# gk969/stm32-speech-recognition

Hardware: AMD Instinct MI355X
Metric: utterances/sec (256-frame, 100 templates) (higher is better)
Workload: dtype int32

## Files before the change

stm32_speech_recognition_amd/csrc/k_mfcc.hip:

```cpp
#include "sr_fft_dev.h"

#ifndef SR_MEL_CHUNKED
#define SR_MEL_CHUNKED 1
#endif

namespace sr {

constexpr int kMfccWaves = 4;
constexpr int kFramesPerWave = 16, kFramesPerWaveMid = 4, kFramesPerWaveSmall = 1;
#ifndef SR_MAG_TAB_BINS
#define SR_MAG_TAB_BINS 8
#endif
constexpr int mfcc_tab_bins(int fpw) { return fpw == kFramesPerWave ? SR_MAG_TAB_BINS : 0; }
static_assert(SR_MAG_TAB_BINS == 0 || SR_MAG_TAB_BINS == 4 || SR_MAG_TAB_BINS == 8, "table bins per lane");
constexpr int kMelPad = kMel + 1;
__device__ __forceinline__ constexpr int mel_chunk_word(int j) { return 256 * ((j >> 2) & 1) + 4 * ((j >> 3) ^ (4 * ((j >> 2) & 1))) + (j & 3); }
constexpr int mfcc_wave_lds_words(int fpw) { return kXchgWords + fpw * kMelPad + 64; }

template <typename Base>
struct MfccTabArgs : Base {
    const uint16_t *mag_q;
    uint32_t mag_table_off;
};
template <typename Base>
constexpr int mfcc_feat_kind<MfccTabArgs<Base>> = mfcc_feat_kind<Base>;
template <typename Base>
static MfccTabArgs<Base> mfcc_tab_args(const Base &b, const MfccMagTab &tab)
{
    MfccTabArgs<Base> r;
    static_cast<Base &>(r) = b;
    r.mag_q = tab.mag_q;
    r.mag_table_off = tab.mag_table_off;
    return r;
}

template <int kFPW, typename Args = MfccTabArgs<MfccArgs>>
__global__ void __launch_bounds__(64 * kMfccWaves, 4) k_mfcc(const Args a)
{
    constexpr int kFeat = mfcc_feat_kind<Args>;
    constexpr uint32_t kFeatW = (kFeat == SR_FEAT_FFT || kFeat == SR_FEAT_MAG) ? kBins : kMel;
    constexpr int kWaveLdsWords = mfcc_wave_lds_words(kFPW);
    constexpr int kTabBins = mfcc_tab_bins(kFPW);
    extern __shared__ __attribute__((aligned(16))) uint32_t smem[];
    __shared__ uint32_t s_dctM[kCoef * kMelPad];
    __shared__ int s_dctS[kCoef * kMelPad];
    __shared__ u32x4 s_tw3[kTw3Row * 4], s_tw5[8 * 64];
    __shared__ u32x4 s_tm[4 * 64];
    const int lane = threadIdx.x & 63, w = __builtin_amdgcn_readfirstlane(threadIdx.x >> 6);
    uint32_t *buf = smem + w * kWaveLdsWords;
    uint32_t *xw = buf;
    uint32_t *powb = buf + kXchgWords, *moff = powb + kFPW * kMelPad;

    for (int i = threadIdx.x; i < kCoef * kMel; i += blockDim.x) {
        const int c = a.t.dct[i], o = (i / kMel) * kMelPad + i % kMel;
        s_dctM[o] = (uint32_t)(((c < 0 ? -c : c) * 262144 + 99) / 100);
        s_dctS[o] = (c > 0) - (c < 0);
    }
    __syncthreads();

    LaneTw tw;
    load_lane_tw(a.t, lane, tw);
    if (w == 0 && lane < 4) {
        const uint32_t *f = &tw.s3[0][0][0];
#pragma unroll
        for (int c = 0; c < 8; c++) s_tw3[lane * kTw3Row + c] = u32x4{f[4 * c], f[4 * c + 1], f[4 * c + 2], f[4 * c + 3]};
    }
    if (w == 1 % kMfccWaves) store_tw32(s_tw5, lane, tw.s5);
#ifndef SR_INJECT_LDS_RACE
    if (w == 2 % kMfccWaves) {
#pragma unroll
        for (int c = 0; c < 2; c++) {
            s_tm[64 * c + lane] = *(const u32x4 *)(a.t.tri_even_m + 8 * lane + 4 * c);
            s_tm[64 * (c + 2) + lane] = *(const u32x4 *)(a.t.tri_odd_m + 8 * lane + 4 * c);
        }
    }
#endif
    __syncthreads();
#ifdef SR_INJECT_LDS_RACE
    if (w == 2 % kMfccWaves) {
#if SR_INJECT_LDS_RACE >= 2
        __builtin_amdgcn_s_sleep(127);
#endif
#pragma unroll
        for (int c = 0; c < 2; c++) {
            s_tm[64 * c + lane] = *(const u32x4 *)(a.t.tri_even_m + 8 * lane + 4 * c);
            s_tm[64 * (c + 2) + lane] = *(const u32x4 *)(a.t.tri_odd_m + 8 * lane + 4 * c);
        }
    }
#endif
    int hamm_m[3];
#pragma unroll
    for (int k = 0; k < 3; k++) hamm_m[k] = (lane + 64 * k < kFrameLen) ? hamm_fused_multiplier(a.t.hamm[lane + 64 * k]) : 0;
    int f_lo = 0, p_hi = 0, p_lo = 0, x_hi = 0, x_lo = 0;
    if (lane < kMel) {
        const int h = lane;
        f_lo = (h == 0) ? 0 : (int)a.t.tri_cen[h - 1];
        const int f_hi = (h == kMel - 1) ? kBins : (int)a.t.tri_cen[h + 1];
        const int ih = f_hi - 1, il = f_lo ? f_lo - 1 : 0, half = (h & 1) ? kBins : 0;
#if SR_MEL_CHUNKED
        p_hi = half + mel_chunk_word(ih), x_hi = (ih >> 3) > 0 ? (ih >> 3) - 1 : 0;
        p_lo = half + mel_chunk_word(il), x_lo = (il >> 3) > 0 ? (il >> 3) - 1 : 0;
#else
        p_hi = half + ih, x_hi = (ih >> 3) > 0 ? (ih >> 3) - 1 : 0;
        p_lo = half + il, x_lo = (il >> 3) > 0 ? (il >> 3) - 1 : 0;
#endif
    }
    const uint64_t mag_p = (uint64_t)a.mag_q;
    const u32x4 mag_rs = {(uint32_t)mag_p, (uint32_t)(mag_p >> 32) | (2u << 16), kMagTabEntries, 0x00027000u};
    const uint32_t tw_off = 32u * (uint32_t)lane;
#if SR_MEL_CHUNKED
    const int e_base = mel_chunk_word(lane);
    constexpr int kEs = 32, kEh = 128;
    const int c0 = mel_chunk_word(8 * lane), c1 = mel_chunk_word(8 * lane + 4);
#else
    const int e_base = lane;
    constexpr int kEs = 64, kEh = 256;
    const int c0 = 8 * lane, c1 = 8 * lane + 4;
#endif

    uint32_t item = blockIdx.x;
    uint32_t nx_nfrm = 0;
    int nx_mid = 0, nx_seg0 = 0;
    if (item < a.n_items) {
        const sr_vad_rec *rec = a.vad + item / a.tiles;
        nx_nfrm = rec->frm_num;
        nx_mid = (int)rec->atap.mid_val;
        nx_seg0 = rec->seg[0];
    }
    for (; item < a.n_items; item += gridDim.x) {
        const uint32_t b = item / a.tiles, tile = item - b * a.tiles;
        const uint32_t nfrm = nx_nfrm;
        const int mid = nx_mid, seg0 = nx_seg0;
        if (item + gridDim.x < a.n_items) {
            const sr_vad_rec *rec = a.vad + (item + gridDim.x) / a.tiles;
            nx_nfrm = rec->frm_num;
            nx_mid = (int)rec->atap.mid_val;
            nx_seg0 = rec->seg[0];
        }
        const uint16_t *row = a.pcm + (uint64_t)b * a.pcm_stride;
        int16_t *out = a.mfcc + (uint64_t)b * a.max_frames * kCoef;
        const uint32_t f0 = tile * (kMfccWaves * kFPW) + w * kFPW;
        uint32_t *frow = nullptr;
        if constexpr (kFeat != 0) frow = a.feat + (uint64_t)b * a.max_frames * kFeatW;
        uint32_t nf = 0;
        if (f0 < nfrm) nf = (nfrm - f0 < (uint32_t)kFPW) ? nfrm - f0 : (uint32_t)kFPW;

        uint32_t s_pp[3] = {0, 0, 0};
        if (nf) {
            const uint16_t *x = row + seg0 + (int)kHop * (int)f0;
#pragma unroll
            for (int k = 0; k < 3; k++) {
                const int i = lane + 64 * k;
                if (i < kFrameLen) s_pp[k] = *(const u32_align2 *)(x + i - 1);
            }
        }
        for (uint32_t fi = 0; fi < nf; fi++) {
#pragma unroll
            for (int k = 0; k < 3; k++) {
                const int i = lane + 64 * k;
                if (i < kFrameLen) xw[i] = k == 0 ? window_sample<4>(s_pp[k], mid, hamm_m[k]) : window_sample<2>(s_pp[k], mid, hamm_m[k]);
            }
            if (fi + 1 < nf) {
                const uint16_t *x = row + seg0 + (int)kHop * (int)(f0 + fi + 1);
#pragma unroll
                for (int k = 0; k < 3; k++) {
                    const int i = lane + 64 * k;
                    if (i < kFrameLen) s_pp[k] = *(const u32_align2 *)(x + i - 1);
                }
            }
            wave_sync();
            uint32_t v[4][4], u[4][4];
            fft_front_real160(xw, lane, tw, s_tw3, v);
            fft_exchange(buf, lane, v, u);
#pragma unroll
            for (int e4 = 0; e4 < 4; e4++)
                bfly_pk<false>(u[0][e4], u[1][e4], u[2][e4], u[3][e4], tw.s4[0][0], tw.s4[0][1], tw.s4[1][0], tw.s4[1][1],
                               tw.s4[2][0], tw.s4[2][1], tw.s4[3][0], tw.s4[3][1]);
            wave_sync();
            uint32_t k5[4][4][2];
            load_tw32(s_tw5, lane, k5);
            uint32_t nn[8];
#pragma unroll
            for (int e3 = 0; e3 < 4; e3++) {
                bfly_pk<true>(u[e3][0], u[e3][1], u[e3][2], u[e3][3], k5[e3][0][0], k5[e3][0][1], k5[e3][1][0],
                              k5[e3][1][1], k5[e3][2][0], k5[e3][2][1], k5[e3][3][0], k5[e3][3][1]);
                if constexpr (kFeat == SR_FEAT_FFT) {
                    uint32_t *fr = frow + (f0 + fi) * kFeatW + lane + 64 * e3;
                    fr[0] = u[e3][0];
                    fr[256] = u[e3][1];
                }
                nn[2 * e3] = (uint32_t)sdot2z(u[e3][0], u[e3][0]);
                nn[2 * e3 + 1] = (uint32_t)sdot2z(u[e3][1], u[e3][1]);
            }
            const uint32_t nmax = max(max(max(max(nn[0], nn[1]), nn[2]), max(max(nn[3], nn[4]), nn[5])), max(nn[6], nn[7]));
#ifdef SR_TESTING
            const bool quiet = __builtin_expect(__builtin_amdgcn_ballot_w64(nmax > kMagSmallMax) == 0 && !a.mag_table_off, 1);
#else
            const bool quiet = __builtin_expect(__builtin_amdgcn_ballot_w64(nmax > kMagSmallMax) == 0, 1);
#endif
            u32x4 tw_e[2], tw_o[2];
            bool cheap = true;
            if (!quiet) {
#pragma unroll
                for (int c = 0; c < 2; c++) {
                    tw_e[c] = *(const u32x4 *)((const char *)a.t.tri_even32 + tw_off + 16 * c);
                    tw_o[c] = *(const u32x4 *)((const char *)a.t.tri_odd32 + tw_off + 16 * c);
                }
                cheap = __builtin_amdgcn_ballot_w64(nmax > a.mag_cheap_max) == 0;
            } else {
                asm volatile("" : "=v"(tw_e[0]), "=v"(tw_e[1]), "=v"(tw_o[0]), "=v"(tw_o[1]));
            }
            uint32_t *eb = buf + e_base;
            if (kTabBins > 0 && quiet) {
                uint32_t tq[8];
#pragma unroll
                for (int e3 = 0; e3 < 4; e3++) {
                    if constexpr (kTabBins == 8)
                        asm volatile("buffer_load_ushort %0, %1, %2, 0 idxen" : "=v"(tq[2 * e3]) : "v"(nn[2 * e3]), "s"(mag_rs));
                    asm volatile("buffer_load_ushort %0, %1, %2, 0 idxen" : "=v"(tq[2 * e3 + 1]) : "v"(nn[2 * e3 + 1]), "s"(mag_rs));
                }
                uint32_t q0s[4];
                if constexpr (kTabBins == 4) {
#pragma unroll
                    for (int e3 = 0; e3 < 4; e3++) q0s[e3] = cvt_u32(__builtin_amdgcn_sqrtf((float)(int)nn[2 * e3]) * 10.0f) << 2;
                }
                if constexpr (kTabBins == 8)
                    asm volatile("s_waitcnt vmcnt(0)" : "+v"(tq[0]), "+v"(tq[1]), "+v"(tq[2]), "+v"(tq[3]), "+v"(tq[4]), "+v"(tq[5]), "+v"(tq[6]), "+v"(tq[7]));
                else
                    asm volatile("s_waitcnt vmcnt(0)" : "+v"(tq[1]), "+v"(tq[3]), "+v"(tq[5]), "+v"(tq[7]));
#pragma unroll
                for (int e3 = 0; e3 < 4; e3++) {
                    uint32_t q0, q1 = tq[2 * e3 + 1];
                    if constexpr (kTabBins == 8) q0 = tq[2 * e3];
                    else q0 = q0s[e3];
                    if constexpr (kFeat == SR_FEAT_MAG) {
                        uint32_t *fr = frow + (f0 + fi) * kFeatW + lane + 64 * e3;
                        fr[0] = q0 >> 2;
                        fr[256] = q1 >> 2;
                    }
                    eb[kEs * e3] = umul24(q0, q0);
                    eb[kEs * e3 + kEh] = umul24(q1, q1);
                }
            } else if (cheap) {
#pragma unroll
                for (int e3 = 0; e3 < 4; e3++) {
                    const f32x2 m = f32x2{__builtin_amdgcn_sqrtf((float)(int)nn[2 * e3]), __builtin_amdgcn_sqrtf((float)(int)nn[2 * e3 + 1])} *
                                    f32x2{10.0f, 10.0f};
                    const uint32_t m0 = cvt_u32(m.x), m1 = cvt_u32(m.y);
                    if constexpr (kFeat == SR_FEAT_MAG) {
                        uint32_t *fr = frow + (f0 + fi) * kFeatW + lane + 64 * e3;
                        fr[0] = m0;
                        fr[256] = m1;
                    }
                    eb[kEs * e3] = umul24(m0, m0);
                    eb[kEs * e3 + kEh] = umul24(m1, m1);
                }
            } else {
#pragma unroll
                for (int e3 = 0; e3 < 4; e3++) {
                    const f32x2 m = sqrt_rn_int2(f32x2{(float)(int)nn[2 * e3], (float)(int)nn[2 * e3 + 1]}) * f32x2{10.0f, 10.0f};
                    const uint32_t m0 = cvt_u32(m.x), m1 = cvt_u32(m.y);
                    if constexpr (kFeat == SR_FEAT_MAG) {
                        uint32_t *fr = frow + (f0 + fi) * kFeatW + lane + 64 * e3;
                        fr[0] = m0;
                        fr[256] = m1;
                    }
                    eb[kEs * e3] = umul24(m0, m0);
                    eb[kEs * e3 + kEh] = umul24(m1, m1);
                }
            }
            wave_sync();
            uint32_t pe[8], po[8], xe, xo;
            {
                const uint4 q0 = *(const uint4 *)(buf + c0), q1 = *(const uint4 *)(buf + c1);
                const uint32_t e[8] = {q0.x, q0.y, q0.z, q0.w, q1.x, q1.y, q1.z, q1.w};
                uint32_t se = 0, so = 0;
                if (quiet) {
#pragma unroll
                    for (int c = 0; c < 2; c++) {
                        const u32x4 me = s_tm[64 * c + lane], mo = s_tm[64 * (c + 2) + lane];
#pragma unroll
                        for (int k = 0; k < 4; k++) {
                            const uint32_t es = kTabBins > 0 ? e[4 * c + k] : e[4 * c + k] << 4;
                            se += mel_term_fused(es, me[k]);
                            so += mel_term_fused(es, mo[k]);
                            pe[4 * c + k] = se;
                            po[4 * c + k] = so;
                        }
                    }
                } else {
#pragma unroll
                    for (int c = 0; c < 2; c++) {
#pragma unroll
                        for (int k = 0; k < 4; k++) {
                            se += e[4 * c + k] * tw_e[c][k] / 100u;
                            so += e[4 * c + k] * tw_o[c][k] / 100u;
                            pe[4 * c + k] = se;
                            po[4 * c + k] = so;
                        }
                    }
                }
                xe = wave_scan_incl(se);
                xo = wave_scan_incl(so);
            }
            *(uint4 *)(buf + c0) = make_uint4(pe[0], pe[1], pe[2], pe[3]);
            *(uint4 *)(buf + c1) = make_uint4(pe[4], pe[5], pe[6], pe[7]);
            *(uint4 *)(buf + kBins + c0) = make_uint4(po[0], po[1], po[2], po[3]);
            *(uint4 *)(buf + kBins + c1) = make_uint4(po[4], po[5], po[6], po[7]);
            buf[2 * kBins + lane] = xe;
            moff[lane] = xo;
            wave_sync();
            if (lane < kMel) {
                const uint32_t *X = (lane & 1) ? moff : buf + 2 * kBins;
                const uint32_t hi = buf[p_hi] + X[x_hi], lo = f_lo ? buf[p_lo] + X[x_lo] : 0u;
                powb[fi * kMelPad + lane] = hi - lo;
                if constexpr (kFeat == SR_FEAT_MEL) frow[(f0 + fi) * kFeatW + lane] = hi - lo;
            }
            wave_sync();
        }

        {
            constexpr int kLogRounds = (kFPW * kMelPad + 63) / 64;
            const uint32_t n_log = nf * kMelPad;
            uint32_t nv[kLogRounds], mv[kLogRounds];
            u32x2 tv[kLogRounds];
#pragma unroll
            for (int r = 0; r < kLogRounds; r++) {
                const uint32_t t = lane + 64u * r;
                nv[r] = powb[t];
                mv[r] = log100_est(nv[r]);
                tv[r] = *(const u32_pair_align4 *)((const char *)a.t.log_thr + 4u * mv[r]);
            }
#pragma unroll
            for (int r = 0; r < kLogRounds; r++) {
                const uint32_t t = lane + 64u * r;
                if (t < n_log) powb[t] = log100_fix(nv[r], mv[r], tv[r].x, tv[r].y) << 14;
            }
        }
        wave_sync();
        if constexpr (kFeat == SR_FEAT_LOGMEL) {
            uint32_t *fw = frow + f0 * kFeatW;
            for (uint32_t t = lane; t < nf * kFeatW; t += 64) {
                const uint32_t fi = t / kFeatW, h = t - fi * kFeatW;
                fw[t] = powb[fi * kMelPad + h] >> 14;
            }
        }
        {
            int16_t *out_w = out + (size_t)f0 * kCoef;
#pragma unroll
            for (uint32_t t = lane; t < (uint32_t)(kFPW * kCoef); t += 64) {
                if (t < nf * kCoef) {
                    const uint32_t fi = umul24(t, 10923u) >> 17, h = t - umul24(fi, (uint32_t)kCoef);
                    const uint32_t *pw = powb + umul24(fi, (uint32_t)kMelPad), *dm = s_dctM + umul24(h, (uint32_t)kMelPad);
                    const int *ds = s_dctS + umul24(h, (uint32_t)kMelPad);
                    int acc = 0;
#pragma unroll
                    for (int i = 0; i < kMel; i++) acc = mad24((int)__umulhi(pw[i], dm[i]), ds[i], acc);
                    out_w[t] = (int16_t)acc;
                }
            }
        }
        wave_sync();
        {
            const uint32_t r0 = f0 + nf, r1 = (f0 + kFPW < a.max_frames) ? f0 + kFPW : a.max_frames;
            for (uint32_t t = r0 * kCoef + lane; t < r1 * kCoef && r0 < r1; t += 64) out[t] = 0;
        }
        if constexpr (kFeat != 0) {
            const uint32_t r0 = f0 + nf, r1 = (f0 + kFPW < a.max_frames) ? f0 + kFPW : a.max_frames;
            for (uint32_t t = r0 * kFeatW + lane; t < r1 * kFeatW && r0 < r1; t += 64) frow[t] = 0;
        }
    }
}

uint32_t mfcc_ext_frames_per_tile();
int mfcc_ext_occupancy(int *per_cu);
void launch_mfcc_ext(const MfccArgs &a, uint32_t grid, hipStream_t s);
void launch_mfcc_ext_features(const MfccArgs &a, int kind, uint32_t *feat, uint32_t grid, hipStream_t s);

uint32_t mfcc_frames_per_tile(uint32_t frame_len) { return frame_len == 320 ? mfcc_ext_frames_per_tile() : (uint32_t)(kMfccWaves * kFramesPerWave); }
uint32_t mfcc_frames_per_tile_small(uint32_t frame_len, uint32_t which)
{
    return frame_len == 320 ? mfcc_ext_frames_per_tile() : (uint32_t)(kMfccWaves * (which ? kFramesPerWaveSmall : kFramesPerWaveMid));
}

uint32_t mfcc_resident_workgroups(uint32_t frame_len)
{
    int dev = 0, n_cu = 0, per_cu = 0;
    if (hipGetDevice(&dev) != hipSuccess) return 0;
    if (hipDeviceGetAttribute(&n_cu, hipDeviceAttributeMultiprocessorCount, dev) != hipSuccess || n_cu < 1) return 0;
    int e;
    if (frame_len == 320)
        e = mfcc_ext_occupancy(&per_cu);
    else
        e = (int)hipOccupancyMaxActiveBlocksPerMultiprocessor(&per_cu, k_mfcc<kFramesPerWave>, 64 * kMfccWaves,
                                                              (size_t)kMfccWaves * mfcc_wave_lds_words(kFramesPerWave) * sizeof(uint32_t));
    if (e != (int)hipSuccess || per_cu < 1) return 0;
    return (uint32_t)(per_cu * n_cu);
}

void launch_mfcc(const MfccArgs &a, const MfccMagTab &tab, hipStream_t s)
{
    if (a.generic) {
        launch_mfcc_gen(a, s);
        return;
    }
    if (a.n_items == 0) return;
    const uint32_t cap = a.grid_cap ? a.grid_cap : 4096u;
    const uint32_t grid = a.n_items < cap ? a.n_items : cap;
    if (a.frame_len == 320) {
        launch_mfcc_ext(a, grid, s);
        return;
    }
    if (a.small_tiles == 2) {
        const size_t lds = (size_t)kMfccWaves * mfcc_wave_lds_words(kFramesPerWaveSmall) * sizeof(uint32_t);
        hipLaunchKernelGGL(k_mfcc<kFramesPerWaveSmall>, dim3(grid), dim3(64 * kMfccWaves), lds, s, mfcc_tab_args(a, tab));
        return;
    }
    if (a.small_tiles == 1) {
        const size_t lds = (size_t)kMfccWaves * mfcc_wave_lds_words(kFramesPerWaveMid) * sizeof(uint32_t);
        hipLaunchKernelGGL(k_mfcc<kFramesPerWaveMid>, dim3(grid), dim3(64 * kMfccWaves), lds, s, mfcc_tab_args(a, tab));
        return;
    }
    const size_t lds = (size_t)kMfccWaves * mfcc_wave_lds_words(kFramesPerWave) * sizeof(uint32_t);
    hipLaunchKernelGGL(k_mfcc<kFramesPerWave>, dim3(grid), dim3(64 * kMfccWaves), lds, s, mfcc_tab_args(a, tab));
}

template <int kFPW, int kKind>
static void launch_mfcc_feat_kind(const MfccArgs &a, const MfccMagTab &tab, uint32_t *feat, uint32_t grid, hipStream_t s)
{
    const size_t lds = (size_t)kMfccWaves * mfcc_wave_lds_words(kFPW) * sizeof(uint32_t);
    hipLaunchKernelGGL((k_mfcc<kFPW, MfccTabArgs<MfccFeatArgs<kKind>>>), dim3(grid), dim3(64 * kMfccWaves), lds, s,
                       mfcc_tab_args(mfcc_feat_args<kKind>(a, feat), tab));
}
template <int kFPW>
static void launch_mfcc_feat_form(const MfccArgs &a, const MfccMagTab &tab, int kind, uint32_t *feat, uint32_t grid, hipStream_t s)
{
    switch (kind) {
    case SR_FEAT_FFT: launch_mfcc_feat_kind<kFPW, SR_FEAT_FFT>(a, tab, feat, grid, s); break;
    case SR_FEAT_MAG: launch_mfcc_feat_kind<kFPW, SR_FEAT_MAG>(a, tab, feat, grid, s); break;
    case SR_FEAT_MEL: launch_mfcc_feat_kind<kFPW, SR_FEAT_MEL>(a, tab, feat, grid, s); break;
    case SR_FEAT_LOGMEL: launch_mfcc_feat_kind<kFPW, SR_FEAT_LOGMEL>(a, tab, feat, grid, s); break;
    default: break;
    }
}

void launch_mfcc_features(const MfccArgs &a, const MfccMagTab &tab, int kind, uint32_t *feat, hipStream_t s)
{
    if (a.generic) {
        launch_mfcc_gen_features(a, kind, feat, s);
        return;
    }
    if (a.n_items == 0) return;
    const uint32_t cap = a.grid_cap ? a.grid_cap : 4096u;
    const uint32_t grid = a.n_items < cap ? a.n_items : cap;
    if (a.frame_len == 320)
        launch_mfcc_ext_features(a, kind, feat, grid, s);
    else if (a.small_tiles == 2)
        launch_mfcc_feat_form<kFramesPerWaveSmall>(a, tab, kind, feat, grid, s);
    else if (a.small_tiles == 1)
        launch_mfcc_feat_form<kFramesPerWaveMid>(a, tab, kind, feat, grid, s);
    else
        launch_mfcc_feat_form<kFramesPerWave>(a, tab, kind, feat, grid, s);
}

}
```

Before: 3.214 million.

## Software-pipeline MFCC frame loop to overlap magnitude table loads with next FFT

```diff
diff --git a/stm32_speech_recognition_amd/csrc/k_mfcc.hip b/stm32_speech_recognition_amd/csrc/k_mfcc.hip
--- a/stm32_speech_recognition_amd/csrc/k_mfcc.hip
+++ b/stm32_speech_recognition_amd/csrc/k_mfcc.hip
@@ -1,4 +1,6 @@
 #include "sr_fft_dev.h"
+
+#include <type_traits>
 
 #ifndef SR_MEL_CHUNKED
 #define SR_MEL_CHUNKED 1
@@ -13,6 +15,17 @@
 #endif
 constexpr int mfcc_tab_bins(int fpw) { return fpw == kFramesPerWave ? SR_MAG_TAB_BINS : 0; }
 static_assert(SR_MAG_TAB_BINS == 0 || SR_MAG_TAB_BINS == 4 || SR_MAG_TAB_BINS == 8, "table bins per lane");
+#ifndef SR_MFCC_PIPE
+#define SR_MFCC_PIPE 1
+#endif
+#ifndef SR_MFCC_PIPE_PEEL
+#define SR_MFCC_PIPE_PEEL 1
+#endif
+#ifndef SR_MFCC_PIPE_VMCNT
+#define SR_MFCC_PIPE_VMCNT (SR_MFCC_PIPE_PEEL ? 3 : 0)
+#endif
+static_assert(SR_MFCC_PIPE_VMCNT == 0 || (SR_MFCC_PIPE_VMCNT == 3 && SR_MFCC_PIPE_PEEL), "younger loads counted by the wait");
+constexpr bool mfcc_pipelined(int fpw) { return SR_MFCC_PIPE && mfcc_tab_bins(fpw) == 8; }
 constexpr int kMelPad = kMel + 1;
 __device__ __forceinline__ constexpr int mel_chunk_word(int j) { return 256 * ((j >> 2) & 1) + 4 * ((j >> 3) ^ (4 * ((j >> 2) & 1))) + (j & 3); }
 constexpr int mfcc_wave_lds_words(int fpw) { return kXchgWords + fpw * kMelPad + 64; }
@@ -41,6 +54,7 @@
     constexpr uint32_t kFeatW = (kFeat == SR_FEAT_FFT || kFeat == SR_FEAT_MAG) ? kBins : kMel;
     constexpr int kWaveLdsWords = mfcc_wave_lds_words(kFPW);
     constexpr int kTabBins = mfcc_tab_bins(kFPW);
+    constexpr bool kPipe = mfcc_pipelined(kFPW);
     extern __shared__ __attribute__((aligned(16))) uint32_t smem[];
     __shared__ uint32_t s_dctM[kCoef * kMelPad];
     __shared__ int s_dctS[kCoef * kMelPad];
@@ -154,6 +168,7 @@
                 if (i < kFrameLen) s_pp[k] = *(const u32_align2 *)(x + i - 1);
             }
         }
+        if constexpr (!kPipe)
         for (uint32_t fi = 0; fi < nf; fi++) {
 #pragma unroll
             for (int k = 0; k < 3; k++) {
@@ -317,6 +332,193 @@
                 if constexpr (kFeat == SR_FEAT_MEL) frow[(f0 + fi) * kFeatW + lane] = hi - lo;
             }
             wave_sync();
+        } else {
+            uint32_t mq[8] = {0, 0, 0, 0, 0, 0, 0, 0};
+            bool pq = true;
+            auto window = [&]() {
+#pragma unroll
+                for (int k = 0; k < 3; k++) {
+                    const int i = lane + 64 * k;
+                    if (i < kFrameLen) xw[i] = k == 0 ? window_sample<4>(s_pp[k], mid, hamm_m[k]) : window_sample<2>(s_pp[k], mid, hamm_m[k]);
+                }
+            };
+            auto request = [&](uint32_t f) {
+                const uint16_t *x = row + seg0 + (int)kHop * (int)(f0 + f);
+#pragma unroll
+                for (int k = 0; k < 3; k++) {
+                    const int i = lane + 64 * k;
+                    if (i < kFrameLen) s_pp[k] = *(const u32_align2 *)(x + i - 1);
+                }
+            };
+            auto middle = [&](uint32_t fi, uint32_t (&v)[4][4], bool more) {
+                uint32_t u[4][4];
+                fft_exchange(buf, lane, v, u);
+#pragma unroll
+                for (int e4 = 0; e4 < 4; e4++)
+                    bfly_pk<false>(u[0][e4], u[1][e4], u[2][e4], u[3][e4], tw.s4[0][0], tw.s4[0][1], tw.s4[1][0], tw.s4[1][1],
+                                   tw.s4[2][0], tw.s4[2][1], tw.s4[3][0], tw.s4[3][1]);
+                wave_sync();
+                uint32_t k5[4][4][2];
+                load_tw32(s_tw5, lane, k5);
+                uint32_t nn[8];
+#pragma unroll
+                for (int e3 = 0; e3 < 4; e3++) {
+                    bfly_pk<true>(u[e3][0], u[e3][1], u[e3][2], u[e3][3], k5[e3][0][0], k5[e3][0][1], k5[e3][1][0],
+                                  k5[e3][1][1], k5[e3][2][0], k5[e3][2][1], k5[e3][3][0], k5[e3][3][1]);
+                    if constexpr (kFeat == SR_FEAT_FFT) {
+                        uint32_t *fr = frow + (f0 + fi) * kFeatW + lane + 64 * e3;
+                        fr[0] = u[e3][0];
+                        fr[256] = u[e3][1];
+                    }
+                    nn[2 * e3] = (uint32_t)sdot2z(u[e3][0], u[e3][0]);
+                    nn[2 * e3 + 1] = (uint32_t)sdot2z(u[e3][1], u[e3][1]);
+                }
+                const uint32_t nmax = max(max(max(max(nn[0], nn[1]), nn[2]), max(max(nn[3], nn[4]), nn[5])), max(nn[6], nn[7]));
+                if (more) {
+                    wave_sync();
+                    window();
+                }
+#ifdef SR_TESTING
+                const bool quiet = __builtin_expect(__builtin_amdgcn_ballot_w64(nmax > kMagSmallMax) == 0 && !a.mag_table_off, 1);
+#else
+                const bool quiet = __builtin_expect(__builtin_amdgcn_ballot_w64(nmax > kMagSmallMax) == 0, 1);
+#endif
+                if (quiet) {
+#pragma unroll
+                    for (int k = 0; k < 8; k++) asm volatile("buffer_load_ushort %0, %1, %2, 0 idxen" : "=v"(mq[k]) : "v"(nn[k]), "s"(mag_rs));
+                } else if (__builtin_amdgcn_ballot_w64(nmax > a.mag_cheap_max) == 0) {
+#pragma unroll
+                    for (int e3 = 0; e3 < 4; e3++) {
+                        const f32x2 m = f32x2{__builtin_amdgcn_sqrtf((float)(int)nn[2 * e3]), __builtin_amdgcn_sqrtf((float)(int)nn[2 * e3 + 1])} *
+                                        f32x2{10.0f, 10.0f};
+                        mq[2 * e3] = cvt_u32(m.x);
+                        mq[2 * e3 + 1] = cvt_u32(m.y);
+                    }
+                } else {
+#pragma unroll
+                    for (int e3 = 0; e3 < 4; e3++) {
+                        const f32x2 m = sqrt_rn_int2(f32x2{(float)(int)nn[2 * e3], (float)(int)nn[2 * e3 + 1]}) * f32x2{10.0f, 10.0f};
+                        mq[2 * e3] = cvt_u32(m.x);
+                        mq[2 * e3 + 1] = cvt_u32(m.y);
+                    }
+                }
+                pq = quiet;
+                if (fi + 2 < nf) request(fi + 2);
+            };
+            auto back_end = [&](uint32_t r, auto young) {
+                wave_sync();
+                auto energies = [&]() {
+                    uint32_t *eb = buf + e_base;
+#pragma unroll
+                    for (int e3 = 0; e3 < 4; e3++) {
+                        const uint32_t q0 = mq[2 * e3], q1 = mq[2 * e3 + 1];
+                        if constexpr (kFeat == SR_FEAT_MAG) {
+                            uint32_t *fr = frow + (f0 + r) * kFeatW + lane + 64 * e3;
+                            const uint32_t sh = pq ? 2u : 0u;
+                            fr[0] = q0 >> sh;
+                            fr[256] = q1 >> sh;
+                        }
+                        eb[kEs * e3] = umul24(q0, q0);
+                        eb[kEs * e3 + kEh] = umul24(q1, q1);
+                    }
+                    wave_sync();
+                };
+                uint32_t pe[8], po[8], se = 0, so = 0;
+                if (pq) {
+                    if constexpr (decltype(young)::value)
+                        asm volatile("s_waitcnt vmcnt(3)" : "+v"(mq[0]), "+v"(mq[1]), "+v"(mq[2]), "+v"(mq[3]), "+v"(mq[4]), "+v"(mq[5]), "+v"(mq[6]), "+v"(mq[7]));
+                    else
+                        asm volatile("s_waitcnt vmcnt(0)" : "+v"(mq[0]), "+v"(mq[1]), "+v"(mq[2]), "+v"(mq[3]), "+v"(mq[4]), "+v"(mq[5]), "+v"(mq[6]), "+v"(mq[7]));
+                    energies();
+                    const uint4 q0 = *(const uint4 *)(buf + c0), q1 = *(const uint4 *)(buf + c1);
+                    const uint32_t e[8] = {q0.x, q0.y, q0.z, q0.w, q1.x, q1.y, q1.z, q1.w};
+#pragma unroll
+                    for (int c = 0; c < 2; c++) {
+                        const u32x4 me = s_tm[64 * c + lane], mo = s_tm[64 * (c + 2) + lane];
+#pragma unroll
+                        for (int k = 0; k < 4; k++) {
+                            se += mel_term_fused(e[4 * c + k], me[k]);
+                            so += mel_term_fused(e[4 * c + k], mo[k]);
+                            pe[4 * c + k] = se;
+                            po[4 * c + k] = so;
+                        }
+                    }
+                } else {
+                    u32x4 tw_e[2], tw_o[2];
+                    uint32_t off = tw_off;
+                    asm("" : "+v"(off));
+#pragma unroll
+                    for (int c = 0; c < 2; c++) {
+                        tw_e[c] = *(const u32x4 *)((const char *)a.t.tri_even32 + off + 16 * c);
+                        tw_o[c] = *(const u32x4 *)((const char *)a.t.tri_odd32 + off + 16 * c);
+                    }
+                    energies();
+                    const uint4 q0 = *(const uint4 *)(buf + c0), q1 = *(const uint4 *)(buf + c1);
+                    const uint32_t e[8] = {q0.x, q0.y, q0.z, q0.w, q1.x, q1.y, q1.z, q1.w};
+#pragma unroll
+                    for (int c = 0; c < 2; c++) {
+#pragma unroll
+                        for (int k = 0; k < 4; k++) {
+                            se += e[4 * c + k] * tw_e[c][k] / 100u;
+                            so += e[4 * c + k] * tw_o[c][k] / 100u;
+                            pe[4 * c + k] = se;
+                            po[4 * c + k] = so;
+                        }
+                    }
+                }
+                const uint32_t xe = wave_scan_incl(se), xo = wave_scan_incl(so);
+                *(uint4 *)(buf + c0) = make_uint4(pe[0], pe[1], pe[2], pe[3]);
+                *(uint4 *)(buf + c1) = make_uint4(pe[4], pe[5], pe[6], pe[7]);
+                *(uint4 *)(buf + kBins + c0) = make_uint4(po[0], po[1], po[2], po[3]);
+                *(uint4 *)(buf + kBins + c1) = make_uint4(po[4], po[5], po[6], po[7]);
+                buf[2 * kBins + lane] = xe;
+                moff[lane] = xo;
+                wave_sync();
+                if (lane < kMel) {
+                    const uint32_t *X = (lane & 1) ? moff : buf + 2 * kBins;
+                    const uint32_t hi = buf[p_hi] + X[x_hi], lo = f_lo ? buf[p_lo] + X[x_lo] : 0u;
+                    powb[r * kMelPad + lane] = hi - lo;
+                    if constexpr (kFeat == SR_FEAT_MEL) frow[(f0 + r) * kFeatW + lane] = hi - lo;
+                }
+                wave_sync();
+            };
+            constexpr std::false_type kDrain{};
+            if (nf) {
+                window();
+                if (nf > 1) request(1);
+#if SR_MFCC_PIPE_PEEL
+                constexpr std::integral_constant<bool, SR_MFCC_PIPE_VMCNT != 0> kSteady{};
+                {
+                    wave_sync();
+                    uint32_t v[4][4];
+                    fft_front_real160(xw, lane, tw, s_tw3, v);
+                    middle(0, v, nf > 1);
+                }
+                for (uint32_t fi = 1; fi + 1 < nf; fi++) {
+                    wave_sync();
+                    uint32_t v[4][4];
+                    fft_front_real160(xw, lane, tw, s_tw3, v);
+                    back_end(fi - 1, kSteady);
+                    middle(fi, v, true);
+                }
+                if (nf > 1) {
+                    wave_sync();
+                    uint32_t v[4][4];
+                    fft_front_real160(xw, lane, tw, s_tw3, v);
+                    back_end(nf - 2, kDrain);
+                    middle(nf - 1, v, false);
+                }
+#else
+                for (uint32_t fi = 0; fi < nf; fi++) {
+                    wave_sync();
+                    uint32_t v[4][4];
+                    fft_front_real160(xw, lane, tw, s_tw3, v);
+                    if (fi > 0) back_end(fi - 1, kDrain);
+                    middle(fi, v, fi + 1 < nf);
+                }
+#endif
+                back_end(nf - 1, kDrain);
+            }
         }
 
         {
@@ -348,7 +550,9 @@
         {
             int16_t *out_w = out + (size_t)f0 * kCoef;
 #pragma unroll
-            for (uint32_t t = lane; t < (uint32_t)(kFPW * kCoef); t += 64) {
+            for (uint32_t tl = lane; tl < (uint32_t)(kFPW * kCoef); tl += 64) {
+                uint32_t t = tl;
+                if constexpr (kPipe) asm volatile("" : "+v"(t));
                 if (t < nf * kCoef) {
                     const uint32_t fi = umul24(t, 10923u) >> 17, h = t - umul24(fi, (uint32_t)kCoef);
                     const uint32_t *pw = powb + umul24(fi, (uint32_t)kMelPad), *dm = s_dctM + umul24(h, (uint32_t)kMelPad);
```

New measurement: 3.266 million (median of 6 runs). +1.6%, better.
